# andrewmilson/ministark

Hardware: NVIDIA B200
Metric: ntt_field_ops_per_s (higher is better)
Workload: dtype u64

## Files before the change

ministark_b200/csrc/api_core.cu:

```cuda
#include <cstring>

#include "ctx.cuh"

namespace ms {

int fail(ms_ctx *c, int code, const char *fmt, ...) {
    char buf[512];
    va_list ap;
    va_start(ap, fmt);
    vsnprintf(buf, sizeof buf, fmt, ap);
    va_end(ap);
    if (c) c->err = buf;
    return code;
}

int scratch_get(ms_ctx *c, int slot, size_t bytes, void **out) {
    Scratch &s = c->scratch[slot];
    if (s.cap < bytes) {
        if (s.ptr) {
            MS_CUDA(c, cudaStreamSynchronize(c->stream));
            MS_CUDA(c, cudaFree(s.ptr));
            s.ptr = nullptr;
            s.cap = 0;
        }
        size_t want = bytes + (bytes >> 3);
        cudaError_t e = cudaMalloc(&s.ptr, want);
        if (e != cudaSuccess) {
            want = bytes;
            e = cudaMalloc(&s.ptr, want);
        }
        if (e != cudaSuccess) {
            s.ptr = nullptr;
            cudaGetLastError();
            return fail(c, MS_ERR_NOMEM, "scratch %d: cudaMalloc(%zu) failed: %s", slot, bytes, cudaGetErrorString(e));
        }
        s.cap = want;
    }
    *out = s.ptr;
    return MS_OK;
}

bool is_device_ptr(const void *p) {
    cudaPointerAttributes a;
    if (cudaPointerGetAttributes(&a, p) != cudaSuccess) {
        cudaGetLastError();
        return false;
    }
    return a.type == cudaMemoryTypeDevice || a.type == cudaMemoryTypeManaged;
}

Staged::Staged(ms_ctx *c, const void *p, size_t nbytes, bool copy_in, bool copy_out_)
    : ctx(c), user(const_cast<void *>(p)), dev(nullptr), bytes(nbytes), staged(false), copy_out(copy_out_), rc(MS_OK) {
    cudaSetDevice(c->device);
    if (p == nullptr || nbytes == 0 || is_device_ptr(p)) {
        dev = user;
        return;
    }
    staged = true;
    cudaError_t e = cudaMalloc(&dev, nbytes);
    if (e != cudaSuccess) {
        cudaGetLastError();
        dev = nullptr;
        rc = fail(c, MS_ERR_NOMEM, "staging cudaMalloc(%zu): %s", nbytes, cudaGetErrorString(e));
        return;
    }
    if (copy_in) {
        e = cudaMemcpyAsync(dev, user, nbytes, cudaMemcpyHostToDevice, c->stream);
        if (e != cudaSuccess) rc = fail(c, MS_ERR_CUDA, "staging H2D: %s", cudaGetErrorString(e));
    }
}
int Staged::finish() {
    if (!staged || dev == nullptr) return rc;
    if (rc == MS_OK && copy_out) {
        cudaError_t e = cudaMemcpyAsync(user, dev, bytes, cudaMemcpyDeviceToHost, ctx->stream);
        if (e != cudaSuccess) rc = fail(ctx, MS_ERR_CUDA, "staging D2H: %s", cudaGetErrorString(e));
    }
    cudaError_t e = cudaStreamSynchronize(ctx->stream);
    if (e != cudaSuccess && rc == MS_OK) rc = fail(ctx, MS_ERR_CUDA, "staging sync: %s", cudaGetErrorString(e));
    cudaFree(dev);
    dev = nullptr;
    return rc;
}
Staged::~Staged() {
    if (staged && dev) {
        cudaStreamSynchronize(ctx->stream);
        cudaFree(dev);
    }
}

__global__ void fill_random_kernel(u64 *dst, size_t n, u64 seed) {
    size_t i = blockIdx.x * (size_t)blockDim.x + threadIdx.x;
    if (i >= n) return;
    u64 s = seed ^ (0xD1B54A32D192ED03ULL * (u64)(i + 1));
    u64 z;
    do {
        s += 0x9E3779B97F4A7C15ULL;
        z = s;
        z = (z ^ (z >> 30)) * 0xBF58476D1CE4E5B9ULL;
        z = (z ^ (z >> 27)) * 0x94D049BB133111EBULL;
        z ^= z >> 31;
    } while (z >= gl::P);
    dst[i] = gl::to_mont(z);
}

template <int EW>
__global__ void bit_reverse_kernel(u64 *data, unsigned log_n, size_t col_stride_words) {
    size_t i = blockIdx.x * (size_t)blockDim.x + threadIdx.x;
    size_t n = (size_t)1 << log_n;
    if (i >= n) return;
    size_t j = log_n ? (__brevll(i) >> (64 - log_n)) : 0;
    if (j <= i) return;
    u64 *col = data + (size_t)blockIdx.y * col_stride_words;
#pragma unroll
    for (int w = 0; w < EW; w++) {
        u64 a = col[i * EW + w], b = col[j * EW + w];
        col[i * EW + w] = b;
        col[j * EW + w] = a;
    }
}

}

using namespace ms;

extern "C" {

const char *ms_version(void) { return "ministark_b200 0.1 (sm_100a)"; }

int ms_ctx_create(int device, ms_ctx **out) {
    if (!out) return MS_ERR_INVALID;
    *out = nullptr;
    int count = 0;
    if (cudaGetDeviceCount(&count) != cudaSuccess || count == 0) {
        cudaGetLastError();
        return MS_ERR_NODEVICE;
    }
    if (device < 0 || device >= count) return MS_ERR_INVALID;
    if (cudaSetDevice(device) != cudaSuccess) return MS_ERR_CUDA;
    ms_ctx *c = new ms_ctx();
    c->device = device;
    if (cudaStreamCreateWithFlags(&c->own_stream, cudaStreamNonBlocking) != cudaSuccess) {
        delete c;
        return MS_ERR_CUDA;
    }
    c->stream = c->own_stream;
    {
        std::vector<u64> h(2 * 4096);
        u64 w = gl::to_mont(1753635133440165772ULL);
        for (int i = 12; i < 32; i++) w = gl::sqr(w);
        u64 wi = gl::inv(w);
        u64 a = gl::ONE, b = gl::ONE;
        for (int e = 0; e < 4096; e++) {
            h[e] = a;
            h[4096 + e] = b;
            a = gl::mul(a, w);
            b = gl::mul(b, wi);
        }
        u64 *d = nullptr;
        if (cudaMalloc(&d, h.size() * 8) != cudaSuccess ||
            cudaMemcpy(d, h.data(), h.size() * 8, cudaMemcpyHostToDevice) != cudaSuccess) {
            delete c;
            return MS_ERR_CUDA;
        }
        c->t4096[0] = d;
        c->t4096[1] = d + 4096;
    }
    if (cudaGetLastError() != cudaSuccess) {
        delete c;
        return MS_ERR_CUDA;
    }
    *out = c;
    return MS_OK;
}

int ms_ctx_destroy(ms_ctx *c) {
    if (!c) return MS_ERR_INVALID;
    cudaSetDevice(c->device);
    cudaStreamSynchronize(c->stream);
    c->plans.clear();
    for (auto &t : c->tw_tables) cudaFree(t.second);
    for (auto &e : c->ptr_tables) cudaFree(e.dev);
    c->ptr_tables.clear();
    c->tw_tables.clear();
    for (auto &s : c->scratch)
        if (s.ptr) cudaFree(s.ptr);
    if (c->t4096[0]) cudaFree(c->t4096[0]);
    if (c->own_stream) cudaStreamDestroy(c->own_stream);
    delete c;
    return MS_OK;
}

int ms_ctx_set_stream(ms_ctx *c, void *s) {
    if (!c) return MS_ERR_INVALID;
    cudaStreamSynchronize(c->stream);
    c->stream = s ? (cudaStream_t)s : c->own_stream;
    return MS_OK;
}

int ms_ctx_sync(ms_ctx *c) {
    if (!c) return MS_ERR_INVALID;
    MS_CUDA(c, cudaStreamSynchronize(c->stream));
    return MS_OK;
}

int ms_set_option(ms_ctx *c, const char *name, int64_t value) {
    if (!name) return MS_ERR_INVALID;
    if (!strcmp(name, "ntt_tma")) { msntt::tma_configure(value ? 1 : 0, 0, 0); return MS_OK; }
    if (!strcmp(name, "ntt_tma_groups")) {
        if (value != 2 && value != 3) return fail(c, MS_ERR_INVALID, "ntt_tma_groups must be 2 or 3");
        msntt::tma_configure(-1, (int)value, 0);
        return MS_OK;
    }
    if (!strcmp(name, "ntt_tma_stages")) {
        if (value < 3 || value > 8) return fail(c, MS_ERR_INVALID, "ntt_tma_stages must be in [3, 8]");
        msntt::tma_configure(-1, 0, (int)value);
        return MS_OK;
    }
    if (!strcmp(name, "drop_plans")) {
        if (!c) return MS_ERR_INVALID;
        cudaSetDevice(c->device);
        ms::ntt_drop_plans(c);
        return MS_OK;
    }
    return fail(c, MS_ERR_INVALID, "unknown option %s", name);
}

const char *ms_last_error(ms_ctx *c) { return c ? c->err.c_str() : "null context"; }
uint64_t ms_launch_count(ms_ctx *c) { return c ? c->launches : 0; }

int ms_alloc_device(ms_ctx *c, size_t bytes, void **out) {
    if (!c || !out) return MS_ERR_INVALID;
    cudaSetDevice(c->device);
    cudaError_t e = cudaMalloc(out, bytes ? bytes : 1);
    if (e != cudaSuccess) {
        cudaGetLastError();
        return fail(c, MS_ERR_NOMEM, "cudaMalloc(%zu): %s", bytes, cudaGetErrorString(e));
    }
    return MS_OK;
}
int ms_alloc_host_pinned(ms_ctx *c, size_t bytes, void **out) {
    if (!c || !out) return MS_ERR_INVALID;
    cudaError_t e = cudaMallocHost(out, bytes ? bytes : 1);
    if (e != cudaSuccess) {
        cudaGetLastError();
        return fail(c, MS_ERR_NOMEM, "cudaMallocHost(%zu): %s", bytes, cudaGetErrorString(e));
    }
    return MS_OK;
}
int ms_free(ms_ctx *c, void *p) {
    if (!c) return MS_ERR_INVALID;
    if (!p) return MS_OK;
    cudaPointerAttributes a;
    if (cudaPointerGetAttributes(&a, p) != cudaSuccess) {
        cudaGetLastError();
        return fail(c, MS_ERR_INVALID, "ms_free: unknown pointer");
    }
    MS_CUDA(c, cudaStreamSynchronize(c->stream));
    if (a.type == cudaMemoryTypeHost)
        MS_CUDA(c, cudaFreeHost(p));
    else if (a.type == cudaMemoryTypeDevice || a.type == cudaMemoryTypeManaged)
        MS_CUDA(c, cudaFree(p));
    else
        return fail(c, MS_ERR_INVALID, "ms_free: not a CUDA allocation");
    return MS_OK;
}
int ms_copy(ms_ctx *c, void *dst, const void *src, size_t bytes) {
    if (!c) return MS_ERR_INVALID;
    MS_CUDA(c, cudaMemcpyAsync(dst, src, bytes, cudaMemcpyDefault, c->stream));
    MS_CUDA(c, cudaStreamSynchronize(c->stream));
    return MS_OK;
}

int ms_fill_random(ms_ctx *c, void *dst, size_t nwords, uint64_t seed) {
    if (!c || !dst) return MS_ERR_INVALID;
    Staged d(c, dst, nwords * 8, false, true);
    if (d.rc) return d.rc;
    if (nwords) {
        fill_random_kernel<<<(unsigned)((nwords + 255) / 256), 256, 0, c->stream>>>(d.as<u64>(), nwords, seed);
        c->launches++;
        MS_CHECK_LAUNCH(c);
    }
    return d.finish();
}

int ms_bit_reverse(ms_ctx *c, int field, void *data, size_t col_stride_elems, unsigned ncols, unsigned log_n) {
    if (!c || !data || (field != MS_FIELD_FP && field != MS_FIELD_FQ3) || log_n > 32 || ncols == 0)
        return fail(c, MS_ERR_INVALID, "ms_bit_reverse: bad argument");
    const size_t n = (size_t)1 << log_n;
    if (ncols > 1 && col_stride_elems < n) return fail(c, MS_ERR_INVALID, "ms_bit_reverse: stride < n");
    const size_t span = ((size_t)(ncols - 1) * col_stride_elems + n) * field * 8;
    Staged d(c, data, span, true, true);
    if (d.rc) return d.rc;
    dim3 grid((unsigned)((n + 255) / 256), ncols);
    if (field == MS_FIELD_FP)
        bit_reverse_kernel<1><<<grid, 256, 0, c->stream>>>(d.as<u64>(), log_n, col_stride_elems);
    else
        bit_reverse_kernel<3><<<grid, 256, 0, c->stream>>>(d.as<u64>(), log_n, col_stride_elems * 3);
    c->launches++;
    MS_CHECK_LAUNCH(c);
    return d.finish();
}

}
```

ministark_b200/csrc/ctx.cuh:

```cuda
#pragma once
#include <cuda_runtime.h>

#include <cstdarg>
#include <cstdint>
#include <cstdio>
#include <deque>
#include <map>
#include <memory>
#include <string>
#include <tuple>
#include <vector>

#include "../../include/ministark_b200.h"
#include "ntt.cuh"

namespace ms {

using gl::u32;
using gl::u64;

struct NttPlanDev;

struct Scratch {
    void *ptr = nullptr;
    size_t cap = 0;
};

}

namespace ms {
struct PtrTable {
    std::vector<void *> host;
    void *dev = nullptr;
};
}

struct ms_ctx {
    int device = 0;
    cudaStream_t own_stream = nullptr;
    cudaStream_t stream = nullptr;
    std::string err;
    uint64_t launches = 0;
    ms::Scratch scratch[4];
    ms::u64 *t4096[2] = {nullptr, nullptr};
    std::map<std::tuple<int, unsigned, int, uint64_t, unsigned, int>, std::shared_ptr<ms::NttPlanDev>> plans;
    std::deque<ms::PtrTable> ptr_tables;
    std::map<unsigned, ms::u64 *> tw_tables;
};

namespace ms {

int fail(ms_ctx *c, int code, const char *fmt, ...);
#define MS_CUDA(ctx, expr)                                                                          \
    do {                                                                                            \
        cudaError_t _e = (expr);                                                                    \
        if (_e != cudaSuccess) return ms::fail(ctx, MS_ERR_CUDA, "%s: %s", #expr, cudaGetErrorString(_e)); \
    } while (0)
#define MS_CHECK_LAUNCH(ctx) MS_CUDA(ctx, cudaGetLastError())

int scratch_get(ms_ctx *c, int slot, size_t bytes, void **out);
bool is_device_ptr(const void *p);

struct Staged {
    ms_ctx *ctx;
    void *user;
    void *dev;
    size_t bytes;
    bool staged, copy_out;
    int rc;
    Staged(ms_ctx *c, const void *p, size_t bytes, bool copy_in, bool copy_out);
    ~Staged();
    int finish();
    template <class T>
    T *as() { return reinterpret_cast<T *>(dev); }
};

struct NttJob {
    int field;
    unsigned log_n;
    bool inverse;
    bool bitrev_out;
    unsigned log_blowup;
    u64 offset;
};
int ntt_get_plan(ms_ctx *c, const NttJob &job, std::shared_ptr<NttPlanDev> *out);
int ntt_plan_tables(ms_ctx *c, unsigned log_n, const u64 **tw_lo, const u64 **tw_hi, u32 *hi_len);
void ntt_drop_plans(ms_ctx *c);
struct LdeScatter {
    u64 *const *block_ptr;
    size_t block_col_stride_words;
    u64 *const *dup_ptr;
    size_t dup_col_stride_words;
    void *const *host_block_ptr = nullptr;
    void *const *host_dup_ptr = nullptr;
};
int ntt_run(ms_ctx *c, NttPlanDev &plan, const u64 *in, size_t in_col_stride_words, u64 *out,
            size_t out_col_stride_words, unsigned ncols, const LdeScatter *scatter = nullptr);

}
```

ministark_b200/csrc/hash.cu:

```cuda
#include <mutex>
#include <cstring>
#include "ctx.cuh"
#include <algorithm>
#include <cstring>
#include <deque>
#include <vector>

namespace ms {

__constant__ u32 c_K[64] = {
    0x428a2f98, 0x71374491, 0xb5c0fbcf, 0xe9b5dba5, 0x3956c25b, 0x59f111f1, 0x923f82a4, 0xab1c5ed5,
    0xd807aa98, 0x12835b01, 0x243185be, 0x550c7dc3, 0x72be5d74, 0x80deb1fe, 0x9bdc06a7, 0xc19bf174,
    0xe49b69c1, 0xefbe4786, 0x0fc19dc6, 0x240ca1cc, 0x2de92c6f, 0x4a7484aa, 0x5cb0a9dc, 0x76f988da,
    0x983e5152, 0xa831c66d, 0xb00327c8, 0xbf597fc7, 0xc6e00bf3, 0xd5a79147, 0x06ca6351, 0x14292967,
    0x27b70a85, 0x2e1b2138, 0x4d2c6dfc, 0x53380d13, 0x650a7354, 0x766a0abb, 0x81c2c92e, 0x92722c85,
    0xa2bfe8a1, 0xa81a664b, 0xc24b8b70, 0xc76c51a3, 0xd192e819, 0xd6990624, 0xf40e3585, 0x106aa070,
    0x19a4c116, 0x1e376c08, 0x2748774c, 0x34b0bcb5, 0x391c0cb3, 0x4ed8aa4a, 0x5b9cca4f, 0x682e6ff3,
    0x748f82ee, 0x78a5636f, 0x84c87814, 0x8cc70208, 0x90befffa, 0xa4506ceb, 0xbef9a3f7, 0xc67178f2};

__device__ __forceinline__ u32 bswap(u32 x) { return __byte_perm(x, 0, 0x0123); }

__device__ __forceinline__ u32 rotr(u32 x, int r) { return __funnelshift_r(x, x, r); }
__device__ __forceinline__ u32 big_sigma1(u32 e) { return rotr(e, 6) ^ rotr(e, 11) ^ rotr(e, 25); }
__device__ __forceinline__ u32 big_sigma0(u32 a) { return rotr(a, 2) ^ rotr(a, 13) ^ rotr(a, 22); }
__device__ __forceinline__ u32 small_sigma0(u32 w) { return rotr(w, 7) ^ rotr(w, 18) ^ (w >> 3); }
__device__ __forceinline__ u32 small_sigma1(u32 w) { return rotr(w, 17) ^ rotr(w, 19) ^ (w >> 10); }

__constant__ u32 c_KW_pad64[64];
struct KW64 {
    u32 v[64];
};

__constant__ u32 c_one = 1;
template <int ON>
__device__ __forceinline__ u32 fma_add(u32 a, u32 b) {
    if constexpr (ON) {
        u32 d;
        asm("mad.lo.u32 %0, %1, %2, %3;" : "=r"(d) : "r"(a), "r"(c_one), "r"(b));
        return d;
    } else {
        return a + b;
    }
}

__constant__ u32 c_pow2[33] = {0, 1u << 31, 1u << 30, 1u << 29, 1u << 28, 1u << 27, 1u << 26, 1u << 25, 1u << 24, 1u << 23, 1u << 22,
                               1u << 21, 1u << 20, 1u << 19, 1u << 18, 1u << 17, 1u << 16, 1u << 15, 1u << 14, 1u << 13, 1u << 12,
                               1u << 11, 1u << 10, 1u << 9, 1u << 8, 1u << 7, 1u << 6, 1u << 5, 1u << 4, 1u << 3, 1u << 2, 1u << 1, 1};
template <int ON, int R>
__device__ __forceinline__ u32 shr_fma(u32 x) {
    if constexpr (ON) {
        u32 d;
        asm("mul.hi.u32 %0, %1, %2;" : "=r"(d) : "r"(x), "r"(c_pow2[R]));
        return d;
    } else {
        return x >> R;
    }
}
template <int V> __device__ __forceinline__ u32 small_sigma0_v(u32 w) { return rotr(w, 7) ^ rotr(w, 18) ^ shr_fma<((V & 16) != 0), 3>(w); }
template <int V> __device__ __forceinline__ u32 small_sigma1_v(u32 w) { return rotr(w, 17) ^ rotr(w, 19) ^ shr_fma<((V & 16) != 0), 10>(w); }

template <int V>
struct ShaT {
    u32 h[8];
    __device__ __forceinline__ void init() {
        h[0] = 0x6a09e667; h[1] = 0xbb67ae85; h[2] = 0x3c6ef372; h[3] = 0xa54ff53a;
        h[4] = 0x510e527f; h[5] = 0x9b05688c; h[6] = 0x1f83d9ab; h[7] = 0x5be0cd19;
    }
    __device__ __forceinline__ void compress(u32 (&w)[16]) {
        u32 a = h[0], b = h[1], c = h[2], d = h[3], e = h[4], f = h[5], g = h[6], hh = h[7];
#pragma unroll
        for (int i = 0; i < 64; i++) {
            if (i >= 16)
                w[i & 15] = fma_add<((V & 1) != 0)>(fma_add<((V & 1) != 0)>(w[i & 15], small_sigma0_v<V>(w[(i + 1) & 15])),
                                              fma_add<((V & 1) != 0)>(w[(i + 9) & 15], small_sigma1_v<V>(w[(i + 14) & 15])));
            u32 ch = (e & f) ^ (~e & g);
            u32 t1 = fma_add<((V & 2) != 0)>(fma_add<((V & 2) != 0)>(hh, big_sigma1(e)), fma_add<((V & 2) != 0)>(ch, fma_add<((V & 8) != 0)>(w[i & 15], c_K[i])));
            u32 mj = (a & b) ^ (a & c) ^ (b & c);
            u32 t2 = fma_add<((V & 4) != 0)>(big_sigma0(a), mj);
            hh = g; g = f; f = e; e = fma_add<((V & 4) != 0)>(d, t1); d = c; c = b; b = a; a = fma_add<((V & 4) != 0)>(t1, t2);
        }
        h[0] += a; h[1] += b; h[2] += c; h[3] += d; h[4] += e; h[5] += f; h[6] += g; h[7] += hh;
    }
    __device__ __forceinline__ void compress_pad64() { compress_const(c_KW_pad64); }
    __device__ __forceinline__ void compress_const(const u32 (&kw)[64]) {
        u32 a = h[0], b = h[1], c = h[2], d = h[3], e = h[4], f = h[5], g = h[6], hh = h[7];
#pragma unroll
        for (int i = 0; i < 64; i++) {
            u32 ch = (e & f) ^ (~e & g);
            u32 t1 = fma_add<((V & 2) != 0)>(fma_add<((V & 2) != 0)>(hh, big_sigma1(e)), fma_add<((V & 8) != 0)>(ch, kw[i]));
            u32 mj = (a & b) ^ (a & c) ^ (b & c);
            u32 t2 = fma_add<((V & 4) != 0)>(big_sigma0(a), mj);
            hh = g; g = f; f = e; e = fma_add<((V & 4) != 0)>(d, t1); d = c; c = b; b = a; a = fma_add<((V & 4) != 0)>(t1, t2);
        }
        h[0] += a; h[1] += b; h[2] += c; h[3] += d; h[4] += e; h[5] += f; h[6] += g; h[7] += hh;
    }
    __device__ __forceinline__ void store(u32 *out) const {
        uint4 lo = make_uint4(bswap(h[0]), bswap(h[1]), bswap(h[2]), bswap(h[3]));
        uint4 hi = make_uint4(bswap(h[4]), bswap(h[5]), bswap(h[6]), bswap(h[7]));
        reinterpret_cast<uint4 *>(out)[0] = lo;
        reinterpret_cast<uint4 *>(out)[1] = hi;
    }
};

using Sha = ShaT<0>;

template <int V>
__global__ void __launch_bounds__(128) hash_rows_kernel(const u64 *__restrict__ cols, size_t col_stride_words,
                                                         unsigned lanes, unsigned words_per_row, size_t nrows,
                                                         u32 *__restrict__ digests, int const_pad,
                                                         const __grid_constant__ KW64 kw_pad) {
    const size_t i = blockIdx.x * (size_t)blockDim.x + threadIdx.x;
    if (i >= nrows) return;
    ShaT<V> s;
    s.init();
    const unsigned msg_words32 = words_per_row * 2;
    const unsigned total32 = ((msg_words32 + 1 + 2 + 15) / 16) * 16;
    const u64 bitlen = (u64)words_per_row * 64;
    const u64 *row = cols + i * lanes;
    unsigned t = 0, cidx = 0, l = 0;
    const unsigned data_blocks = const_pad ? msg_words32 / 16 : total32 / 16;
    for (unsigned blk = 0; blk < data_blocks; blk++) {
        u32 w[16];
#pragma unroll
        for (int j = 0; j < 8; j++) {
            const unsigned g = blk * 16 + 2 * j;
            u32 lo = 0, hi = 0;
            if (t < words_per_row) {
                u64 x = gl::from_mont(row[(size_t)cidx * col_stride_words + l]);
                lo = bswap((u32)x);
                hi = bswap((u32)(x >> 32));
                t++;
                if (++l == lanes) { l = 0; cidx++; }
            } else {
                if (g == msg_words32) lo = 0x80000000u;
                if (g == total32 - 2) { lo = (u32)(bitlen >> 32); hi = (u32)bitlen; }
            }
            w[2 * j] = lo;
            w[2 * j + 1] = hi;
        }
        s.compress(w);
    }
    if (const_pad) s.compress_const(kw_pad.v);
    s.store(digests + i * 8);
}

template <int V>
__global__ void __launch_bounds__(128) merkle_level_kernel(const u32 *__restrict__ src, u32 *__restrict__ dst,
                                                            size_t count) {
    const size_t k = blockIdx.x * (size_t)blockDim.x + threadIdx.x;
    if (k >= count) return;
    ShaT<V> s;
    s.init();
    u32 w[16];
    const uint4 *p = reinterpret_cast<const uint4 *>(src + k * 16);
#pragma unroll
    for (int q = 0; q < 4; q++) {
        uint4 v = p[q];
        w[4 * q] = bswap(v.x); w[4 * q + 1] = bswap(v.y); w[4 * q + 2] = bswap(v.z); w[4 * q + 3] = bswap(v.w);
    }
    s.compress(w);
    s.compress_pad64();
    s.store(dst + k * 8);
}

__global__ void __launch_bounds__(128) pow_grind_kernel(uint4 seed_lo, uint4 seed_hi, unsigned bits, u64 base, u64 count,
                                                         unsigned long long *best) {
    const u64 idx = blockIdx.x * (u64)blockDim.x + threadIdx.x;
    if (idx >= count) return;
    const u64 nonce = base + idx;
    Sha s;
    s.init();
    u32 w[16] = {seed_lo.x, seed_lo.y, seed_lo.z, seed_lo.w, seed_hi.x, seed_hi.y, seed_hi.z, seed_hi.w,
                 (u32)(nonce >> 32), (u32)nonce, 0x80000000u, 0, 0, 0, 0, 320};
    s.compress(w);
    unsigned lz = __clz(s.h[0]);
    if (s.h[0] == 0) { lz = 32 + __clz(s.h[1]); if (s.h[1] == 0) lz = 64 + __clz(s.h[2]); }
    if (lz >= bits) atomicMin(best, (unsigned long long)nonce);
}

__global__ void gather_digests_kernel(const uint4 *__restrict__ leaves, const uint4 *__restrict__ nodes, const u64 *__restrict__ sel,
                                      unsigned count, uint4 *__restrict__ out) {
    const unsigned t = blockIdx.x * blockDim.x + threadIdx.x;
    if (t >= 2 * count) return;
    const u64 s = sel[t >> 1];
    const uint4 *src = (s >> 63) ? nodes : leaves;
    out[t] = src[2 * (s & ~(1ull << 63)) + (t & 1)];
}

static int sha_variant() {
    static int v = -1;
    if (v < 0) {
        const char *e = getenv("MS_SHA_FMA_ADDS");
        v = (e && atoi(e) == 0) ? 0 : 7;
    }
    return v;
}
#define MS_SHA_DISPATCH(KERNEL, GRID, ...)                                        \
    if (sha_variant() == 0) KERNEL<0><<<GRID, 128, 0, c->stream>>>(__VA_ARGS__);   \
    else KERNEL<7><<<GRID, 128, 0, c->stream>>>(__VA_ARGS__);

static int row_pad_schedule(unsigned row_words, KW64 *kw);
static int hash_rows_dev(ms_ctx *c, int field, const u64 *cols, size_t col_stride_elems, unsigned ncols, size_t nrows,
                         u32 *digests) {
    if (nrows == 0) return MS_OK;
    const unsigned threads = 128;
    KW64 kw;
    const int const_pad = row_pad_schedule(ncols * field, &kw);
    MS_SHA_DISPATCH(hash_rows_kernel, (unsigned)((nrows + threads - 1) / threads), cols, col_stride_elems * field, (unsigned)field,
                    ncols * field, nrows, digests, const_pad, kw);
    c->launches++;
    MS_CHECK_LAUNCH(c);
    return MS_OK;
}

static u32 h_rotr(u32 x, int r) { return (x >> r) | (x << (32 - r)); }
static void pad_schedule(unsigned long long bitlen, u32 kw[64]);
static int upload_pad_schedule(ms_ctx *c) {
    static bool done[64] = {false};
    static std::mutex mu;
    std::lock_guard<std::mutex> lock(mu);
    int dev = 0;
    cudaGetDevice(&dev);
    if (dev >= 0 && dev < 64 && done[dev]) return MS_OK;
    u32 kw[64];
    pad_schedule(512, kw);
    MS_CUDA(c, cudaMemcpyToSymbol(c_KW_pad64, kw, sizeof kw));
    if (dev >= 0 && dev < 64) done[dev] = true;
    return MS_OK;
}
static int row_pad_schedule(unsigned row_words, KW64 *kw) {
    memset(kw, 0, sizeof *kw);
    if (row_words % 8) return 0;
    pad_schedule((unsigned long long)row_words * 64, kw->v);
    return 1;
}
static void pad_schedule(unsigned long long bitlen, u32 kw[64]) {
    static const u32 K[64] = {
        0x428a2f98, 0x71374491, 0xb5c0fbcf, 0xe9b5dba5, 0x3956c25b, 0x59f111f1, 0x923f82a4, 0xab1c5ed5,
        0xd807aa98, 0x12835b01, 0x243185be, 0x550c7dc3, 0x72be5d74, 0x80deb1fe, 0x9bdc06a7, 0xc19bf174,
        0xe49b69c1, 0xefbe4786, 0x0fc19dc6, 0x240ca1cc, 0x2de92c6f, 0x4a7484aa, 0x5cb0a9dc, 0x76f988da,
        0x983e5152, 0xa831c66d, 0xb00327c8, 0xbf597fc7, 0xc6e00bf3, 0xd5a79147, 0x06ca6351, 0x14292967,
        0x27b70a85, 0x2e1b2138, 0x4d2c6dfc, 0x53380d13, 0x650a7354, 0x766a0abb, 0x81c2c92e, 0x92722c85,
        0xa2bfe8a1, 0xa81a664b, 0xc24b8b70, 0xc76c51a3, 0xd192e819, 0xd6990624, 0xf40e3585, 0x106aa070,
        0x19a4c116, 0x1e376c08, 0x2748774c, 0x34b0bcb5, 0x391c0cb3, 0x4ed8aa4a, 0x5b9cca4f, 0x682e6ff3,
        0x748f82ee, 0x78a5636f, 0x84c87814, 0x8cc70208, 0x90befffa, 0xa4506ceb, 0xbef9a3f7, 0xc67178f2};
    u32 w[64] = {0};
    w[0] = 0x80000000u;
    w[14] = (u32)(bitlen >> 32);
    w[15] = (u32)bitlen;
    for (int i = 16; i < 64; i++) {
        u32 s0 = h_rotr(w[i - 15], 7) ^ h_rotr(w[i - 15], 18) ^ (w[i - 15] >> 3);
        u32 s1 = h_rotr(w[i - 2], 17) ^ h_rotr(w[i - 2], 19) ^ (w[i - 2] >> 10);
        w[i] = w[i - 16] + s0 + w[i - 7] + s1;
    }
    for (int i = 0; i < 64; i++) kw[i] = K[i] + w[i];
}

static int merkle_nodes_dev(ms_ctx *c, const u32 *leaves, size_t n, u32 *nodes) {
    if (int rc = upload_pad_schedule(c)) return rc;
    MS_CUDA(c, cudaMemsetAsync(nodes, 0, 32, c->stream));
    const unsigned threads = 128;
    MS_SHA_DISPATCH(merkle_level_kernel, (unsigned)((n / 2 + threads - 1) / threads), leaves, nodes + (n / 2) * 8, n / 2);
    c->launches++;
    MS_CHECK_LAUNCH(c);
    for (size_t size = n / 4; size >= 1; size >>= 1) {
        MS_SHA_DISPATCH(merkle_level_kernel, (unsigned)((size + threads - 1) / threads), nodes + 2 * size * 8, nodes + size * 8, size);
        c->launches++;
        MS_CHECK_LAUNCH(c);
    }
    return MS_OK;
}

}

using namespace ms;

extern "C" {

int ms_hash_rows_sha256(ms_ctx *c, int field, const void *cols, size_t col_stride_elems, unsigned ncols, size_t nrows,
                        void *digests) {
    if (!c || !cols || !digests) return MS_ERR_INVALID;
    if (field != MS_FIELD_FP && field != MS_FIELD_FQ3) return fail(c, MS_ERR_INVALID, "unknown field id %d", field);
    if (ncols == 0) return fail(c, MS_ERR_INVALID, "ms_hash_rows_sha256: no columns");
    if (ncols > 1 && col_stride_elems < nrows) return fail(c, MS_ERR_INVALID, "ms_hash_rows_sha256: stride < nrows");
    Staged in(c, cols, ((size_t)(ncols - 1) * col_stride_elems + nrows) * field * 8, true, false);
    if (in.rc) return in.rc;
    Staged out(c, digests, nrows * 32, false, true);
    if (out.rc) return out.rc;
    int rc = hash_rows_dev(c, field, in.as<u64>(), col_stride_elems, ncols, nrows, out.as<u32>());
    if (rc) return rc;
    if ((rc = in.finish())) return rc;
    return out.finish();
}

int ms_merkle_nodes_sha256(ms_ctx *c, const void *leaves, size_t n, void *nodes) {
    if (!c || !leaves || !nodes) return MS_ERR_INVALID;
    if (n < 2 || (n & (n - 1))) return fail(c, MS_ERR_INVALID, "merkle tree needs a power-of-two number of leaves >= 2, got %zu", n);
    Staged in(c, leaves, n * 32, true, false);
    if (in.rc) return in.rc;
    Staged out(c, nodes, n * 32, false, true);
    if (out.rc) return out.rc;
    int rc = merkle_nodes_dev(c, in.as<u32>(), n, out.as<u32>());
    if (rc) return rc;
    if ((rc = in.finish())) return rc;
    return out.finish();
}

int ms_merkle_commit_sha256(ms_ctx *c, int field, const void *cols, size_t col_stride_elems, unsigned ncols, size_t nrows,
                            void *leaves, void *nodes, void *root) {
    if (!c || !cols || !root) return MS_ERR_INVALID;
    if (field != MS_FIELD_FP && field != MS_FIELD_FQ3) return fail(c, MS_ERR_INVALID, "unknown field id %d", field);
    if (ncols == 0) return fail(c, MS_ERR_INVALID, "ms_merkle_commit_sha256: no columns");
    if (nrows < 2 || (nrows & (nrows - 1))) return fail(c, MS_ERR_INVALID, "merkle tree needs a power-of-two number of leaves >= 2, got %zu", nrows);
    if (ncols > 1 && col_stride_elems < nrows) return fail(c, MS_ERR_INVALID, "ms_merkle_commit_sha256: stride < nrows");
    Staged in(c, cols, ((size_t)(ncols - 1) * col_stride_elems + nrows) * field * 8, true, false);
    if (in.rc) return in.rc;
    int rc;
    void *lv = nullptr, *nd = nullptr;
    Staged lout(c, leaves, leaves ? nrows * 32 : 0, false, true);
    if (lout.rc) return lout.rc;
    Staged nout(c, nodes, nodes ? nrows * 32 : 0, false, true);
    if (nout.rc) return nout.rc;
    if (leaves) lv = lout.dev;
    else if ((rc = scratch_get(c, 2, nrows * 32, &lv))) return rc;
    if (nodes) nd = nout.dev;
    else if ((rc = scratch_get(c, 3, nrows * 32, &nd))) return rc;
    if ((rc = hash_rows_dev(c, field, in.as<u64>(), col_stride_elems, ncols, nrows, (u32 *)lv))) return rc;
    if ((rc = merkle_nodes_dev(c, (const u32 *)lv, nrows, (u32 *)nd))) return rc;
    MS_CUDA(c, cudaMemcpyAsync(root, (const char *)nd + 32, 32, cudaMemcpyDefault, c->stream));
    MS_CUDA(c, cudaStreamSynchronize(c->stream));
    if ((rc = in.finish())) return rc;
    if ((rc = lout.finish())) return rc;
    return nout.finish();
}


int ms_merkle_commit_rows_sha256(ms_ctx *c, const void *rows, unsigned row_words, size_t nrows, void *leaves, void *nodes,
                                 void *root) {
    if (!c || !rows || !root || row_words == 0) return MS_ERR_INVALID;
    if (nrows < 2 || (nrows & (nrows - 1))) return fail(c, MS_ERR_INVALID, "merkle tree needs a power-of-two number of leaves >= 2, got %zu", nrows);
    Staged in(c, rows, nrows * row_words * 8, true, false);
    if (in.rc) return in.rc;
    int rc;
    void *lv = nullptr, *nd = nullptr;
    Staged lout(c, leaves, leaves ? nrows * 32 : 0, false, true);
    if (lout.rc) return lout.rc;
    Staged nout(c, nodes, nodes ? nrows * 32 : 0, false, true);
    if (nout.rc) return nout.rc;
    if (leaves) lv = lout.dev;
    else if ((rc = scratch_get(c, 2, nrows * 32, &lv))) return rc;
    if (nodes) nd = nout.dev;
    else if ((rc = scratch_get(c, 3, nrows * 32, &nd))) return rc;
    const unsigned threads = 128;
    KW64 kw;
    const int const_pad = row_pad_schedule(row_words, &kw);
    MS_SHA_DISPATCH(hash_rows_kernel, (unsigned)((nrows + threads - 1) / threads), in.as<u64>(), (size_t)0, row_words, row_words, nrows,
                    (u32 *)lv, const_pad, kw);
    c->launches++;
    MS_CHECK_LAUNCH(c);
    if ((rc = merkle_nodes_dev(c, (const u32 *)lv, nrows, (u32 *)nd))) return rc;
    MS_CUDA(c, cudaMemcpyAsync(root, (const char *)nd + 32, 32, cudaMemcpyDefault, c->stream));
    MS_CUDA(c, cudaStreamSynchronize(c->stream));
    if ((rc = in.finish())) return rc;
    if ((rc = lout.finish())) return rc;
    return nout.finish();
}


int ms_pow_grind_sha256(ms_ctx *c, const uint8_t *seed, unsigned bits, uint64_t *nonce_out) {
    if (!c || !seed || !nonce_out) return MS_ERR_INVALID;
    if (bits > 64) return fail(c, MS_ERR_INVALID, "ms_pow_grind_sha256: at most 64 bits supported");
    cudaSetDevice(c->device);
    u32 sw[8];
    for (int i = 0; i < 8; i++)
        sw[i] = ((u32)seed[4 * i] << 24) | ((u32)seed[4 * i + 1] << 16) | ((u32)seed[4 * i + 2] << 8) | seed[4 * i + 3];
    void *best;
    int rc = scratch_get(c, 3, 64, &best);
    if (rc) return rc;
    const unsigned long long none = ~0ull;
    const u64 batch = 1ull << 24;
    for (u64 base = 1;; base += batch) {
        MS_CUDA(c, cudaMemcpyAsync(best, &none, 8, cudaMemcpyHostToDevice, c->stream));
        pow_grind_kernel<<<(unsigned)(batch / 128), 128, 0, c->stream>>>(make_uint4(sw[0], sw[1], sw[2], sw[3]),
                                                                         make_uint4(sw[4], sw[5], sw[6], sw[7]), bits, base, batch,
                                                                         (unsigned long long *)best);
        c->launches++;
        MS_CHECK_LAUNCH(c);
        unsigned long long got = none;
        MS_CUDA(c, cudaMemcpyAsync(&got, best, 8, cudaMemcpyDeviceToHost, c->stream));
        MS_CUDA(c, cudaStreamSynchronize(c->stream));
        if (got != none) {
            *nonce_out = got;
            return MS_OK;
        }
        if (base > (~0ull) - 2 * batch) return fail(c, MS_ERR_INVALID, "nonce not found");
    }
}

int ms_merkle_prove_sha256(ms_ctx *c, const void *leaves, const void *nodes, size_t n_leaves, const uint64_t *indices,
                           unsigned n_indices, uint8_t *initial_leaves, uint8_t *sibling_leaves, uint8_t *path_nodes,
                           unsigned counts[3]) {
    if (!c || !leaves || !nodes || !indices || !initial_leaves || !sibling_leaves || !path_nodes || !counts) return MS_ERR_INVALID;
    if (n_leaves < 2 || (n_leaves & (n_leaves - 1))) return fail(c, MS_ERR_INVALID, "ms_merkle_prove: leaf count must be a power of two >= 2");
    cudaSetDevice(c->device);
    std::vector<u64> idx(indices, indices + n_indices);
    for (u64 i : idx)
        if (i >= n_leaves) return fail(c, MS_ERR_INVALID, "leaf index `%llu` cannot exceed the number of leaves (`%llu`)",
                                       (unsigned long long)i, (unsigned long long)n_leaves);
    std::sort(idx.begin(), idx.end());
    idx.erase(std::unique(idx.begin(), idx.end()), idx.end());
    const u64 NODE = 1ull << 63;
    std::vector<u64> init, sib, path;
    std::deque<u64> node_q;
    for (size_t k = 0; k < idx.size(); k++) {
        const u64 i = idx[k];
        init.push_back(i);
        node_q.push_back((n_leaves + i) >> 1);
        if (k + 1 < idx.size() && (i ^ 1) == idx[k + 1]) {
            init.push_back(idx[++k]);
            continue;
        }
        sib.push_back(i ^ 1);
    }
    while (!node_q.empty()) {
        const u64 i = node_q.front();
        node_q.pop_front();
        if (i > 2) node_q.push_back(i >> 1);
        if (!node_q.empty() && (i ^ 1) == node_q.front()) {
            node_q.pop_front();
            continue;
        }
        path.push_back((i ^ 1) | NODE);
    }
    counts[0] = (unsigned)init.size();
    counts[1] = (unsigned)sib.size();
    counts[2] = (unsigned)path.size();
    std::vector<u64> sel(init);
    sel.insert(sel.end(), sib.begin(), sib.end());
    sel.insert(sel.end(), path.begin(), path.end());
    const unsigned total = (unsigned)sel.size();
    if (!total) return MS_OK;
    Staged lv(c, leaves, n_leaves * 32, true, false);
    if (lv.rc) return lv.rc;
    Staged nd(c, nodes, n_leaves * 32, true, false);
    if (nd.rc) return nd.rc;
    void *dsel, *dout;
    int rc;
    if ((rc = scratch_get(c, 2, (size_t)total * 8, &dsel))) return rc;
    if ((rc = scratch_get(c, 3, (size_t)total * 32, &dout))) return rc;
    MS_CUDA(c, cudaMemcpyAsync(dsel, sel.data(), (size_t)total * 8, cudaMemcpyHostToDevice, c->stream));
    gather_digests_kernel<<<(2 * total + 127) / 128, 128, 0, c->stream>>>(lv.as<uint4>(), nd.as<uint4>(), (const u64 *)dsel, total,
                                                                           (uint4 *)dout);
    c->launches++;
    MS_CHECK_LAUNCH(c);
    std::vector<uint8_t> host((size_t)total * 32);
    MS_CUDA(c, cudaMemcpyAsync(host.data(), dout, host.size(), cudaMemcpyDeviceToHost, c->stream));
    MS_CUDA(c, cudaStreamSynchronize(c->stream));
    memcpy(initial_leaves, host.data(), init.size() * 32);
    memcpy(sibling_leaves, host.data() + init.size() * 32, sib.size() * 32);
    memcpy(path_nodes, host.data() + (init.size() + sib.size()) * 32, path.size() * 32);
    if ((rc = lv.finish())) return rc;
    return nd.finish();
}

}
```

Baseline: 1347 billion.

## Add specialized SHA leaf kernel and FMA-pipe rotate variants for hashing

Adds a fixed-block-count leaf hashing kernel, on by default, that loads column-strided row words, converts them from Montgomery form and prefetches the next block while compressing. Adds optional variants that compute some SHA rotates with wide multiplies on the FMA pipe to balance ALU pressure, selected through a new option. The old environment-variable dispatch is dropped and the add-on-FMA variant is fixed. The metric measures NTT throughput, so the hashing changes may not affect it.

After: 1288 billion (median of 6 runs). 0.956x the previous value.

```diff
diff --git a/ministark_b200/csrc/api_core.cu b/ministark_b200/csrc/api_core.cu
--- a/ministark_b200/csrc/api_core.cu
+++ b/ministark_b200/csrc/api_core.cu
@@ -214,6 +214,11 @@
     if (!strcmp(name, "ntt_tma_stages")) {
         if (value < 3 || value > 8) return fail(c, MS_ERR_INVALID, "ntt_tma_stages must be in [3, 8]");
         msntt::tma_configure(-1, 0, (int)value);
+        return MS_OK;
+    }
+    if (!strcmp(name, "sha_leaf")) { ms::sha_configure((int)value, -1); return MS_OK; }
+    if (!strcmp(name, "sha_rot")) {
+        if (value < 0 || value > INT32_MAX || ms::sha_configure(-1, (int)value)) return fail(c, MS_ERR_INVALID, "unknown sha_rot variant %lld", (long long)value);
         return MS_OK;
     }
     if (!strcmp(name, "drop_plans")) {
diff --git a/ministark_b200/csrc/ctx.cuh b/ministark_b200/csrc/ctx.cuh
--- a/ministark_b200/csrc/ctx.cuh
+++ b/ministark_b200/csrc/ctx.cuh
@@ -86,6 +86,7 @@
 int ntt_get_plan(ms_ctx *c, const NttJob &job, std::shared_ptr<NttPlanDev> *out);
 int ntt_plan_tables(ms_ctx *c, unsigned log_n, const u64 **tw_lo, const u64 **tw_hi, u32 *hi_len);
 void ntt_drop_plans(ms_ctx *c);
+int sha_configure(int leaf, int rot);
 struct LdeScatter {
     u64 *const *block_ptr;
     size_t block_col_stride_words;
diff --git a/ministark_b200/csrc/hash.cu b/ministark_b200/csrc/hash.cu
--- a/ministark_b200/csrc/hash.cu
+++ b/ministark_b200/csrc/hash.cu
@@ -2,7 +2,7 @@
 #include <cstring>
 #include "ctx.cuh"
 #include <algorithm>
-#include <cstring>
+#include <atomic>
 #include <deque>
 #include <vector>
 
@@ -21,10 +21,6 @@
 __device__ __forceinline__ u32 bswap(u32 x) { return __byte_perm(x, 0, 0x0123); }
 
 __device__ __forceinline__ u32 rotr(u32 x, int r) { return __funnelshift_r(x, x, r); }
-__device__ __forceinline__ u32 big_sigma1(u32 e) { return rotr(e, 6) ^ rotr(e, 11) ^ rotr(e, 25); }
-__device__ __forceinline__ u32 big_sigma0(u32 a) { return rotr(a, 2) ^ rotr(a, 13) ^ rotr(a, 22); }
-__device__ __forceinline__ u32 small_sigma0(u32 w) { return rotr(w, 7) ^ rotr(w, 18) ^ (w >> 3); }
-__device__ __forceinline__ u32 small_sigma1(u32 w) { return rotr(w, 17) ^ rotr(w, 19) ^ (w >> 10); }
 
 __constant__ u32 c_KW_pad64[64];
 struct KW64 {
@@ -56,10 +52,26 @@
         return x >> R;
     }
 }
-template <int V> __device__ __forceinline__ u32 small_sigma0_v(u32 w) { return rotr(w, 7) ^ rotr(w, 18) ^ shr_fma<((V & 16) != 0), 3>(w); }
-template <int V> __device__ __forceinline__ u32 small_sigma1_v(u32 w) { return rotr(w, 17) ^ rotr(w, 19) ^ shr_fma<((V & 16) != 0), 10>(w); }
-
-template <int V>
+
+template <int ON, int R>
+__device__ __forceinline__ u32 rot(u32 x) {
+    if constexpr (ON) {
+        unsigned long long p;
+        asm("mul.wide.u32 %0, %1, %2;" : "=l"(p) : "r"(x), "r"(c_pow2[R]));
+        return fma_add<1>((u32)p, (u32)(p >> 32));
+    } else {
+        return rotr(x, R);
+    }
+}
+
+constexpr int kRotSel[] = {0, 1 | 2, 4 | 8, 1 | 2 | 4 | 8};
+constexpr int kRotVariants = sizeof kRotSel / sizeof kRotSel[0];
+template <int R> __device__ __forceinline__ u32 big_sigma1_r(u32 e) { return rotr(e, 6) ^ rotr(e, 11) ^ rot<(R & 1), 25>(e); }
+template <int R> __device__ __forceinline__ u32 big_sigma0_r(u32 a) { return rotr(a, 2) ^ rotr(a, 13) ^ rot<(R & 2), 22>(a); }
+template <int V, int R> __device__ __forceinline__ u32 small_sigma0_v(u32 w) { return rotr(w, 7) ^ rot<(R & 4), 18>(w) ^ shr_fma<((V & 16) != 0), 3>(w); }
+template <int V, int R> __device__ __forceinline__ u32 small_sigma1_v(u32 w) { return rotr(w, 17) ^ rot<(R & 8), 19>(w) ^ shr_fma<((V & 16) != 0), 10>(w); }
+
+template <int V, int R = 0>
 struct ShaT {
     u32 h[8];
     __device__ __forceinline__ void init() {
@@ -71,12 +83,12 @@
 #pragma unroll
         for (int i = 0; i < 64; i++) {
             if (i >= 16)
-                w[i & 15] = fma_add<((V & 1) != 0)>(fma_add<((V & 1) != 0)>(w[i & 15], small_sigma0_v<V>(w[(i + 1) & 15])),
-                                              fma_add<((V & 1) != 0)>(w[(i + 9) & 15], small_sigma1_v<V>(w[(i + 14) & 15])));
+                w[i & 15] = fma_add<((V & 1) != 0)>(fma_add<((V & 1) != 0)>(w[i & 15], small_sigma0_v<V, R>(w[(i + 1) & 15])),
+                                              fma_add<((V & 1) != 0)>(w[(i + 9) & 15], small_sigma1_v<V, R>(w[(i + 14) & 15])));
             u32 ch = (e & f) ^ (~e & g);
-            u32 t1 = fma_add<((V & 2) != 0)>(fma_add<((V & 2) != 0)>(hh, big_sigma1(e)), fma_add<((V & 2) != 0)>(ch, fma_add<((V & 8) != 0)>(w[i & 15], c_K[i])));
+            u32 t1 = fma_add<((V & 2) != 0)>(fma_add<((V & 2) != 0)>(hh, big_sigma1_r<R>(e)), fma_add<((V & 2) != 0)>(ch, fma_add<((V & 8) != 0)>(w[i & 15], c_K[i])));
             u32 mj = (a & b) ^ (a & c) ^ (b & c);
-            u32 t2 = fma_add<((V & 4) != 0)>(big_sigma0(a), mj);
+            u32 t2 = fma_add<((V & 4) != 0)>(big_sigma0_r<R>(a), mj);
             hh = g; g = f; f = e; e = fma_add<((V & 4) != 0)>(d, t1); d = c; c = b; b = a; a = fma_add<((V & 4) != 0)>(t1, t2);
         }
         h[0] += a; h[1] += b; h[2] += c; h[3] += d; h[4] += e; h[5] += f; h[6] += g; h[7] += hh;
@@ -87,9 +99,9 @@
 #pragma unroll
         for (int i = 0; i < 64; i++) {
             u32 ch = (e & f) ^ (~e & g);
-            u32 t1 = fma_add<((V & 2) != 0)>(fma_add<((V & 2) != 0)>(hh, big_sigma1(e)), fma_add<((V & 8) != 0)>(ch, kw[i]));
+            u32 t1 = fma_add<((V & 2) != 0)>(fma_add<((V & 2) != 0)>(hh, big_sigma1_r<R>(e)), fma_add<((V & 8) != 0)>(ch, kw[i]));
             u32 mj = (a & b) ^ (a & c) ^ (b & c);
-            u32 t2 = fma_add<((V & 4) != 0)>(big_sigma0(a), mj);
+            u32 t2 = fma_add<((V & 4) != 0)>(big_sigma0_r<R>(a), mj);
             hh = g; g = f; f = e; e = fma_add<((V & 4) != 0)>(d, t1); d = c; c = b; b = a; a = fma_add<((V & 4) != 0)>(t1, t2);
         }
         h[0] += a; h[1] += b; h[2] += c; h[3] += d; h[4] += e; h[5] += f; h[6] += g; h[7] += hh;
@@ -104,14 +116,14 @@
 
 using Sha = ShaT<0>;
 
-template <int V>
+template <int V, int R>
 __global__ void __launch_bounds__(128) hash_rows_kernel(const u64 *__restrict__ cols, size_t col_stride_words,
                                                          unsigned lanes, unsigned words_per_row, size_t nrows,
                                                          u32 *__restrict__ digests, int const_pad,
                                                          const __grid_constant__ KW64 kw_pad) {
     const size_t i = blockIdx.x * (size_t)blockDim.x + threadIdx.x;
     if (i >= nrows) return;
-    ShaT<V> s;
+    ShaT<V, R> s;
     s.init();
     const unsigned msg_words32 = words_per_row * 2;
     const unsigned total32 = ((msg_words32 + 1 + 2 + 15) / 16) * 16;
@@ -144,12 +156,53 @@
     s.store(digests + i * 8);
 }
 
-template <int V>
+template <int V, int R, int B, bool ROWS, int P = 0, int M = 1>
+__global__ void __launch_bounds__(128, M) hash_leaf_kernel(const u64 *__restrict__ cols, size_t col_stride_words, size_t nrows,
+                                                         u32 *__restrict__ digests, const __grid_constant__ KW64 kw_pad) {
+    const size_t i = blockIdx.x * (size_t)blockDim.x + threadIdx.x;
+    if (i >= nrows) return;
+    const u64 *p = ROWS ? cols + i * (8 * B) : cols + i;
+    const size_t stride = ROWS ? 1 : col_stride_words;
+    u64 x[8];
+    if constexpr (P == 0) {
+#pragma unroll
+        for (int j = 0; j < 8; j++) x[j] = p[j * stride];
+    }
+    ShaT<V, R> s;
+    s.init();
+#pragma unroll
+    for (int blk = 0; blk < B; blk++) {
+        u32 w[16];
+        if constexpr (P != 0) {
+#pragma unroll
+            for (int j = 0; j < 8; j++) x[j] = p[(size_t)(blk * 8 + j) * stride];
+        }
+#pragma unroll
+        for (int j = 0; j < 8; j++) {
+            const u64 v = gl::from_mont(x[j]);
+            w[2 * j] = bswap((u32)v);
+            w[2 * j + 1] = bswap((u32)(v >> 32));
+        }
+        if (blk + 1 < B) {
+#pragma unroll
+            for (int j = 0; j < 8; j++) {
+                const u64 *q = p + (size_t)((blk + 1) * 8 + j) * stride;
+                if constexpr (P == 0) x[j] = *q;
+                if constexpr (P == 1) asm volatile("prefetch.global.L1 [%0];" ::"l"(q));
+            }
+        }
+        s.compress(w);
+    }
+    s.compress_const(kw_pad.v);
+    s.store(digests + i * 8);
+}
+
+template <int V, int R>
 __global__ void __launch_bounds__(128) merkle_level_kernel(const u32 *__restrict__ src, u32 *__restrict__ dst,
                                                             size_t count) {
     const size_t k = blockIdx.x * (size_t)blockDim.x + threadIdx.x;
     if (k >= count) return;
-    ShaT<V> s;
+    ShaT<V, R> s;
     s.init();
     u32 w[16];
     const uint4 *p = reinterpret_cast<const uint4 *>(src + k * 16);
@@ -187,30 +240,83 @@
     out[t] = src[2 * (s & ~(1ull << 63)) + (t & 1)];
 }
 
-static int sha_variant() {
-    static int v = -1;
-    if (v < 0) {
-        const char *e = getenv("MS_SHA_FMA_ADDS");
-        v = (e && atoi(e) == 0) ? 0 : 7;
-    }
-    return v;
-}
-#define MS_SHA_DISPATCH(KERNEL, GRID, ...)                                        \
-    if (sha_variant() == 0) KERNEL<0><<<GRID, 128, 0, c->stream>>>(__VA_ARGS__);   \
-    else KERNEL<7><<<GRID, 128, 0, c->stream>>>(__VA_ARGS__);
+constexpr int kShaAdds = 7;
+
+static std::atomic<int> g_sha_leaf{1};
+static std::atomic<int> g_sha_rot{0};
+
+int sha_configure(int leaf, int rot) {
+    if (rot >= kRotVariants) return -1;
+    if (leaf >= 0) g_sha_leaf = leaf;
+    if (rot >= 0) g_sha_rot = rot;
+    return 0;
+}
+
+#define MS_SHA_ROT_DISPATCH(FN, ...)                               \
+    switch (g_sha_rot.load(std::memory_order_relaxed)) {           \
+        case 1: FN<kRotSel[1]>(__VA_ARGS__); break;                \
+        case 2: FN<kRotSel[2]>(__VA_ARGS__); break;                \
+        case 3: FN<kRotSel[3]>(__VA_ARGS__); break;                \
+        default: FN<kRotSel[0]>(__VA_ARGS__); break;               \
+    }
+static_assert(kRotVariants == 4, "MS_SHA_ROT_DISPATCH lists every kRotSel entry");
+
+template <int R, int B>
+static void launch_leaf(cudaStream_t st, unsigned grid, bool rows, const u64 *cols, size_t col_stride_words, size_t nrows,
+                        u32 *digests, const KW64 &kw) {
+    if constexpr (R == 0 && B == 4) {
+        switch (g_sha_leaf.load()) {
+            case 2: hash_leaf_kernel<kShaAdds, R, B, false, 1, 12><<<grid, 128, 0, st>>>(cols, col_stride_words, nrows, digests, kw); return;
+            case 3: hash_leaf_kernel<kShaAdds, R, B, false, 1, 10><<<grid, 128, 0, st>>>(cols, col_stride_words, nrows, digests, kw); return;
+            case 4: hash_leaf_kernel<kShaAdds, R, B, false, 0, 10><<<grid, 128, 0, st>>>(cols, col_stride_words, nrows, digests, kw); return;
+            case 5: hash_leaf_kernel<kShaAdds, R, B, false, 2, 10><<<grid, 128, 0, st>>>(cols, col_stride_words, nrows, digests, kw); return;
+            default: break;
+        }
+    }
+    if (rows) hash_leaf_kernel<kShaAdds, R, B, true><<<grid, 128, 0, st>>>(cols, 0, nrows, digests, kw);
+    else hash_leaf_kernel<kShaAdds, R, B, false><<<grid, 128, 0, st>>>(cols, col_stride_words, nrows, digests, kw);
+}
+
+template <int R>
+static void launch_hash_rows_r(cudaStream_t st, unsigned grid, int blocks, bool rows, const u64 *cols, size_t col_stride_words,
+                               unsigned lanes, unsigned row_words, size_t nrows, u32 *digests, int const_pad, const KW64 &kw) {
+    switch (blocks) {
+        case 1: launch_leaf<R, 1>(st, grid, rows, cols, col_stride_words, nrows, digests, kw); break;
+        case 2: launch_leaf<R, 2>(st, grid, rows, cols, col_stride_words, nrows, digests, kw); break;
+        case 3: launch_leaf<R, 3>(st, grid, rows, cols, col_stride_words, nrows, digests, kw); break;
+        case 4: launch_leaf<R, 4>(st, grid, rows, cols, col_stride_words, nrows, digests, kw); break;
+        default:
+            hash_rows_kernel<kShaAdds, R><<<grid, 128, 0, st>>>(cols, col_stride_words, lanes, row_words, nrows, digests, const_pad, kw);
+    }
+}
 
 static int row_pad_schedule(unsigned row_words, KW64 *kw);
-static int hash_rows_dev(ms_ctx *c, int field, const u64 *cols, size_t col_stride_elems, unsigned ncols, size_t nrows,
-                         u32 *digests) {
+static int launch_hash_rows(ms_ctx *c, const u64 *cols, size_t col_stride_words, unsigned lanes, unsigned row_words,
+                            size_t nrows, u32 *digests) {
     if (nrows == 0) return MS_OK;
-    const unsigned threads = 128;
+    const unsigned grid = (unsigned)((nrows + 127) / 128);
     KW64 kw;
-    const int const_pad = row_pad_schedule(ncols * field, &kw);
-    MS_SHA_DISPATCH(hash_rows_kernel, (unsigned)((nrows + threads - 1) / threads), cols, col_stride_elems * field, (unsigned)field,
-                    ncols * field, nrows, digests, const_pad, kw);
+    const int const_pad = row_pad_schedule(row_words, &kw);
+    const bool rows = lanes == row_words;
+    const bool leaf = g_sha_leaf.load(std::memory_order_relaxed) && const_pad && row_words <= 32 && (lanes == 1 || rows);
+    MS_SHA_ROT_DISPATCH(launch_hash_rows_r, c->stream, grid, leaf ? (int)(row_words / 8) : 0, rows, cols, col_stride_words, lanes,
+                        row_words, nrows, digests, const_pad, kw);
     c->launches++;
     MS_CHECK_LAUNCH(c);
     return MS_OK;
+}
+
+static int hash_rows_dev(ms_ctx *c, int field, const u64 *cols, size_t col_stride_elems, unsigned ncols, size_t nrows,
+                         u32 *digests) {
+    return launch_hash_rows(c, cols, col_stride_elems * field, (unsigned)field, ncols * field, nrows, digests);
+}
+
+template <int R>
+static void launch_merkle_level_r(cudaStream_t st, const u32 *src, u32 *dst, size_t count) {
+    merkle_level_kernel<kShaAdds, R><<<(unsigned)((count + 127) / 128), 128, 0, st>>>(src, dst, count);
+}
+static void launch_merkle_level(ms_ctx *c, const u32 *src, u32 *dst, size_t count) {
+    MS_SHA_ROT_DISPATCH(launch_merkle_level_r, c->stream, src, dst, count);
 }
 
 static u32 h_rotr(u32 x, int r) { return (x >> r) | (x << (32 - r)); }
@@ -259,12 +365,11 @@
 static int merkle_nodes_dev(ms_ctx *c, const u32 *leaves, size_t n, u32 *nodes) {
     if (int rc = upload_pad_schedule(c)) return rc;
     MS_CUDA(c, cudaMemsetAsync(nodes, 0, 32, c->stream));
-    const unsigned threads = 128;
-    MS_SHA_DISPATCH(merkle_level_kernel, (unsigned)((n / 2 + threads - 1) / threads), leaves, nodes + (n / 2) * 8, n / 2);
+    launch_merkle_level(c, leaves, nodes + (n / 2) * 8, n / 2);
     c->launches++;
     MS_CHECK_LAUNCH(c);
     for (size_t size = n / 4; size >= 1; size >>= 1) {
-        MS_SHA_DISPATCH(merkle_level_kernel, (unsigned)((size + threads - 1) / threads), nodes + 2 * size * 8, nodes + size * 8, size);
+        launch_merkle_level(c, nodes + 2 * size * 8, nodes + size * 8, size);
         c->launches++;
         MS_CHECK_LAUNCH(c);
     }
@@ -351,13 +456,7 @@
     else if ((rc = scratch_get(c, 2, nrows * 32, &lv))) return rc;
     if (nodes) nd = nout.dev;
     else if ((rc = scratch_get(c, 3, nrows * 32, &nd))) return rc;
-    const unsigned threads = 128;
-    KW64 kw;
-    const int const_pad = row_pad_schedule(row_words, &kw);
-    MS_SHA_DISPATCH(hash_rows_kernel, (unsigned)((nrows + threads - 1) / threads), in.as<u64>(), (size_t)0, row_words, row_words, nrows,
-                    (u32 *)lv, const_pad, kw);
-    c->launches++;
-    MS_CHECK_LAUNCH(c);
+    if ((rc = launch_hash_rows(c, in.as<u64>(), 0, row_words, row_words, nrows, (u32 *)lv))) return rc;
     if ((rc = merkle_nodes_dev(c, (const u32 *)lv, nrows, (u32 *)nd))) return rc;
     MS_CUDA(c, cudaMemcpyAsync(root, (const char *)nd + 32, 32, cudaMemcpyDefault, c->stream));
     MS_CUDA(c, cudaStreamSynchronize(c->stream));
diff --git a/profiles/exp_sha_r03.py b/profiles/exp_sha_r03.py
--- /dev/null
+++ b/profiles/exp_sha_r03.py
@@ -0,0 +1,87 @@
+#!/usr/bin/env python
+import argparse
+import json
+import os
+import statistics
+import subprocess
+import sys
+
+import torch
+
+sys.path.insert(0, os.path.dirname(os.path.dirname(os.path.abspath(__file__))))
+import ministark_b200 as ms
+
+VARIANTS = [(leaf, rot) for leaf in (0, 1) for rot in range(4)]
+
+
+def gpu_info():
+    q = "name,power.limit,clocks.max.sm"
+    out = subprocess.run(["nvidia-smi", f"--query-gpu={q}", "--format=csv,noheader"], capture_output=True, text=True,
+                         check=True).stdout.splitlines()[0]
+    return dict(zip(q.split(","), (v.strip() for v in out.split(","))))
+
+
+def main():
+    ap = argparse.ArgumentParser()
+    ap.add_argument("--log-rows", type=int, default=27)
+    ap.add_argument("--ncols", type=int, default=32)
+    ap.add_argument("--rounds", type=int, default=3)
+    ap.add_argument("--reps", type=int, default=5)
+    ap.add_argument("--warmup", type=int, default=2)
+    ap.add_argument("--out", default=os.path.join(os.path.dirname(os.path.abspath(__file__)), "exp_sha_r03_b200.jsonl"))
+    args = ap.parse_args()
+    info = gpu_info()
+    stream = torch.cuda.Stream()
+    torch.cuda.set_stream(stream)
+    ctx = ms.Context(0, stream=stream.cuda_stream)
+    N, ncols = 1 << args.log_rows, args.ncols
+    lde = torch.empty((ncols, N), dtype=torch.int64, device="cuda")
+    ctx.fill_random(lde, ncols * N, 5)
+    leaves = torch.empty((N, 4), dtype=torch.int64, device="cuda")
+    nodes = torch.empty_like(leaves)
+
+    def timed(fn):
+        for _ in range(args.warmup):
+            fn()
+        a, b = torch.cuda.Event(enable_timing=True), torch.cuda.Event(enable_timing=True)
+        a.record()
+        for _ in range(args.reps):
+            fn()
+        b.record()
+        torch.cuda.synchronize()
+        return a.elapsed_time(b) / args.reps
+
+    rows, bad = [], []
+    base_root = None
+    with open(args.out, "w") as f:
+        for rnd in range(args.rounds):
+            for leaf, rot in VARIANTS:
+                ctx.set_option("sha_leaf", leaf)
+                ctx.set_option("sha_rot", rot)
+                root = ctx.merkle_commit(lde, ms.FP, N, ncols, leaves=leaves, nodes=nodes).hex()
+                base_root = base_root or root
+                leaf_ms = timed(lambda: ctx.hash_rows(lde, leaves, ms.FP, N, ncols))
+                level_ms = timed(lambda: ctx.merkle_nodes(leaves, nodes, N))
+                r = {"round": rnd, "sha_leaf": leaf, "sha_rot": rot, "rows": N, "ncols": ncols, "leaf_ms": round(leaf_ms, 3),
+                     "levels_ms": round(level_ms, 3), "commit_ms": round(leaf_ms + level_ms, 3), "root": root,
+                     "root_ok": root == base_root, **info}
+                rows.append(r)
+                if root != base_root:
+                    bad.append((leaf, rot))
+                f.write(json.dumps(r) + "\n")
+                print(json.dumps(r), flush=True)
+        for leaf, rot in VARIANTS:
+            sel = [r for r in rows if (r["sha_leaf"], r["sha_rot"]) == (leaf, rot)]
+            summ = {"summary": True, "sha_leaf": leaf, "sha_rot": rot, "rounds": len(sel), **info}
+            for k in ("leaf_ms", "levels_ms", "commit_ms"):
+                v = [r[k] for r in sel]
+                summ[k + "_median"] = round(statistics.median(v), 3)
+                summ[k + "_spread"] = round(max(v) - min(v), 3)
+            f.write(json.dumps(summ) + "\n")
+            print(json.dumps(summ), flush=True)
+    if bad:
+        raise SystemExit(f"exp_sha_r03: root differs from the baseline for variants {bad}")
+
+
+if __name__ == "__main__":
+    main()
diff --git a/profiles/sha_sass_count.py b/profiles/sha_sass_count.py
--- /dev/null
+++ b/profiles/sha_sass_count.py
@@ -0,0 +1,54 @@
+#!/usr/bin/env python
+import collections
+import os
+import re
+import subprocess
+import sys
+
+ALU = ("SHF", "LOP3", "IADD3", "IADD", "PRMT", "SEL", "ISETP", "LEA", "MOV", "VIADD")
+
+
+def kernels(path):
+    sass = subprocess.run(["cuobjdump", "-sass", path], capture_output=True, text=True, check=True).stdout
+    out, name = {}, None
+    for line in sass.splitlines():
+        m = re.match(r"\s*Function : (\S+)", line)
+        if m:
+            name = m.group(1)
+            out[name] = collections.Counter()
+            continue
+        m = re.match(r"\s*/\*[0-9a-f]{4,}\*/\s+(?:@!?U?P\w+\s+)?([A-Z0-9_.]+)", line)
+        if m and name:
+            op = m.group(1)
+            base = op.split(".")[0]
+            if base == "IMAD" and (".WIDE" in op or ".HI" in op):
+                base = "IMAD.WIDE" if ".WIDE" in op else "IMAD.HI"
+            out[name][base] += 1
+    return out
+
+
+def pretty(name):
+    d = subprocess.run(["c++filt", name], capture_output=True, text=True).stdout.strip()
+    d = d.replace("ms::", "").replace("void ", "")
+    return d.split("(")[0]
+
+
+def main():
+    here = os.path.dirname(os.path.dirname(os.path.abspath(__file__)))
+    path = sys.argv[1] if len(sys.argv) > 1 else os.path.join(here, "ministark_b200", "csrc", "build", "hash.o")
+    cols = ["SHF", "LOP3", "IADD3", "IMAD", "IMAD.WIDE", "IMAD.HI", "PRMT", "LDG"]
+    print("| kernel | total | ALU pipe | FMA pipe | " + " | ".join(cols) + " |")
+    print("|---|" + "---:|" * (3 + len(cols)))
+    rows = []
+    for name, ops in kernels(path).items():
+        if not any(k in name for k in ("hash_leaf_kernel", "hash_rows_kernel", "merkle_level_kernel")):
+            continue
+        alu = sum(v for k, v in ops.items() if k in ALU)
+        fma = sum(v for k, v in ops.items() if k.startswith("IMAD"))
+        rows.append((pretty(name), sum(ops.values()), alu, fma, [ops.get(k, 0) for k in cols]))
+    for n, tot, alu, fma, c in sorted(rows):
+        print(f"| `{n}` | {tot} | {alu} | {fma} | " + " | ".join(map(str, c)) + " |")
+
+
+if __name__ == "__main__":
+    main()
```
